# PantoMatrix/PantoMatrix

Hardware: NVIDIA H100
Metric: motion_frames_per_sec (higher is better)
Workload: dtype fp16x3 (two fp16 operand planes, 3 products, f32 accumulate)

## Files before the change

include/pm_emage.h:

```cpp
#ifndef PM_EMAGE_H
#define PM_EMAGE_H
#include <stdint.h>
#ifdef __cplusplus
extern "C" {
#endif

#define PM_ABI_VERSION 5
#define PM_FMT_F16 0x100
#define PM_TC_TILE_SHIFT 16
int pm_abi_version(void);
int pm_memset_async(void* ptr, int value, long long bytes, void* stream);
int pm_device_cc(void);

int pm_tapgemm_f32(const float* A, long long a_bs, int lda, int batch, int rows_in, int cin,
                   const float* W, const float* bias, int taps, int stride, int pad,
                   int rows_out, int cout,
                   const float* residual, long long r_bs, int ldr,
                   int act, float slope,
                   float* out, long long o_bs, int ldo, void* stream);

int pm_tapgemm_tc(const uint16_t* A, long long a_ps, long long a_bs, int lda, int batch, int rows_in, int cin,
                  const uint16_t* W, long long w_ps, int w_rows, int ldw, int taps, int pad, int nsplit,
                  const float* bias, int rows_out, int cout,
                  const float* residual, long long r_bs, int ldr,
                  int act, int act_cols, float slope, float acc_scale,
                  float* out_f32, long long o_bs, int ldo,
                  uint16_t* out_bf16, long long ob_ps, long long ob_bs, int ldob, int out_nsplit,
                  const void* prefetch, long long prefetch_bytes, void* stream);

int pm_split_bf16(const float* x, long long x_bs, int ldx, int batch, int rows, int ch,
                  uint16_t* out, long long o_ps, long long o_bs, int ldo, int nsplit, void* stream);

int pm_wav_stem_f32(const float* audio, long long a_bs, long long a_ws, int batch, int windows, int n_samples,
                    const float* w1, const float* b1, const float* wd, const float* bd, int cout,
                    int ksize, int stride, int pad, int rows_out, float slope,
                    float* y1, float* sc,
                    uint16_t* planes, long long p_ps, int p_ld, int p_nsplit, void* stream);

int pm_add_layernorm_f32(const float* x, const float* r, const float* gamma, const float* beta,
                         float* out, long long rows, int ch, float eps,
                         uint16_t* planes, long long p_ps, int p_ld, int p_nsplit, void* stream);

int pm_attention_f32(const float* Q, int ldq, const float* K, int ldk, const float* V, int ldv,
                     float* O, int ldo, int batch, int heads, int tq, int tk, int head_dim,
                     uint16_t* planes, long long p_ps, int p_ld, int p_nsplit, void* stream);

int pm_attention_tc(const uint16_t* Q, long long q_ps, long long q_bs, int ldq, int q_cols, int q_col0,
                    const uint16_t* K, long long k_ps, long long k_bs, int ldk, int k_cols, int k_col0,
                    const uint16_t* V, long long v_ps, long long v_bs, int ldv, int v_cols, int v_col0,
                    float* O, int ldo, int batch, int heads, int tq, int tk, int head_dim,
                    uint16_t* planes, long long p_ps, int p_ld, int p_nsplit, void* stream);

int pm_add_rows_f32(const float* x, const float* pe, const float* spk, int first, int second,
                    float* out, int batch, int rows, int ch,
                    uint16_t* planes, long long p_ps, int p_ld, int p_nsplit, void* stream);
int pm_add2_f32(const float* a, const float* b, float* out, long long n, int ch,
                uint16_t* planes, long long p_ps, int p_ld, int p_nsplit, void* stream);
int pm_add2_strided_f32(const float* a, long long lda, const float* b, long long ldb, float* out, long long ldo,
                        long long rows, long long ch,
                        uint16_t* planes, long long p_ps, int p_ld, int p_nsplit, void* stream);

int pm_window_input_f32(const float* motion, const float* mask, const float* seed, const float* mask_embedding,
                        float* out, int batch, int total_len, int start, int win_len, int pre, int ch, long long seed_bs,
                        uint16_t* planes, long long p_ps, int p_ld, int p_nsplit, void* stream);

int pm_l2_argmin_f32(const float* z, long long rows, int rows_per_batch, long long z_bs,
                     const float* codebook, const float* e2, int n_codes, int e_dim, long long* index, void* stream);
int pm_l2_argmin_tc(const float* z, long long rows, int rows_per_batch, long long z_bs,
                    const float* codebook, const float* e2, int n_codes, int e_dim, long long* index, int max_ctas,
                    void* stream);
int pm_l2_argmin_simt_f32(const float* z, long long rows, int rows_per_batch, long long z_bs,
                          const float* codebook, const float* e2, int n_codes, int e_dim, long long* index, void* stream);
int pm_row_argmax_f32(const float* x, long long rows, int ch, int ldx, int rows_per_batch, long long x_bs,
                      long long* index, int* nonfinite, void* stream);
int pm_gather_rows_f32(const float* codebook, long long n_table, const long long* index, long long rows, int ch,
                       float* out, uint16_t* planes, long long p_ps, int p_ld, int p_nsplit, void* stream);
int pm_row_sqnorm_f32(const float* x, int rows, int ch, float* out, void* stream);

int pm_pose_compose_f32(const float* face, const float* upper, const float* hands, const float* lower,
                        float* expression, float* axis_angle, float* motion4inf, long long bt, void* stream);

int pm_global_trans_f32(const float* rec, int ld, int vel_off, const float* ref_trans, int ref_bs, float dt,
                        float* trans, int batch, int t, void* stream);

int pm_resample_poly_f32(const void* pcm, int is_int16, long long in_bs, int batch, long long n_in, int channels,
                         const float* bank, int up, int down, int taps, long long n_pre_remove,
                         float* out, long long out_bs, void* stream);

int pm_lstm_bidir_f32(const float* xproj, long long x_bs, int ldx, const float* whh,
                      float* y, long long y_bs, int ldy, unsigned int* barrier,
                      int batch, int t, int hidden, void* stream);
int pm_lstm_cond_f32(const float* spk, long long n_spk, int spk_dim, const long long* speaker_id,
// ... 11 lines not shown
```

pantomatrix_b200/csrc/pm_tapgemm_tc.cu:

```cuda
#include <cuda.h>
#include <stdio.h>
#include <stdlib.h>

#include <cstring>
#include "pm_common.cuh"
#include "../../include/pm_emage.h"


namespace {

constexpr int BM = 128;
constexpr int BK = 64;
constexpr int MMA_K = 16;
constexpr int A_TILE_BYTES = BM * BK * 2;
constexpr int PRODUCER_THREADS = 128;
constexpr int CONSUMER_THREADS = 256;
constexpr int NUM_THREADS = PRODUCER_THREADS + CONSUMER_THREADS;
constexpr int PRODUCER_REGS = 40, CONSUMER_REGS = 232;
static_assert(PRODUCER_THREADS * PRODUCER_REGS + CONSUMER_THREADS * CONSUMER_REGS == (65536 / NUM_THREADS & ~7) * NUM_THREADS,
              "the setmaxnreg split must use exactly the launch's register pool");
constexpr int STAMP_WARP = PRODUCER_THREADS / 32;
constexpr int MAX_STAGES = 8;
constexpr int RING_KB = 200;

struct TcParams {
  int taps, pad, nsplit, kblocks;
  int rows_out, cout, batch;
  int R, NB;
  int w_rows;
  const float* bias;
  const float* residual; long long r_bs; int ldr;
  int act, act_cols; float slope;
  float* out_f32; long long o_bs; int ldo;
  __nv_bfloat16* out_bf16; long long ob_ps, ob_bs; int ldob; int out_nsplit;
  int stages;
  const uint8_t* prefetch; long long prefetch_bytes;
  float acc_scale;
};

#ifdef PM_TC_TIMING
__device__ unsigned long long pm_tc_stamps[4096 * 8];
#define PM_STAMP(i)                                                                                              \
  do {                                                                                                           \
    if ((threadIdx.x & 31) == 0) {                                                                               \
      const unsigned cta_ = (blockIdx.z * gridDim.y + blockIdx.y) * gridDim.x + blockIdx.x;                      \
      if (cta_ < 4096) pm_tc_stamps[cta_ * 8 + (i)] = (unsigned long long)clock64();                             \
    }                                                                                                            \
  } while (0)
#else
#define PM_STAMP(i) do {} while (0)
#endif

#include "pm_tc_ptx.cuh"

template <int BN, bool F16>
__device__ __forceinline__ void mma_k16(float (&d)[BN / 2], uint64_t a, uint64_t b) {
  static_assert(BN == 64 || BN == 128, "64- or 128-column tiles (see pm_tapgemm_tc)");
  if constexpr (BN == 64) wgmma_m64n64k16<!F16>(d, a, b);
  else wgmma_m64n128k16<!F16>(d, a, b);
}

template <int BN, bool F16, int NSPLIT>
__device__ __forceinline__ void mma_kblock(float (&main)[BN / 2], float (&corr)[BN / 2], uint64_t a0, uint64_t w0) {
  constexpr uint64_t A_PL = A_TILE_BYTES >> 4, W_PL = (BN * BK * 2) >> 4, K_ST = (MMA_K * 2) >> 4;
  if constexpr (NSPLIT == 3) {
#pragma unroll
    for (int k = 0; k < BK / MMA_K; ++k) mma_k16<BN, F16>(corr, a0 + k * K_ST, w0 + 2 * W_PL + k * K_ST);
#pragma unroll
    for (int k = 0; k < BK / MMA_K; ++k) mma_k16<BN, F16>(corr, a0 + A_PL + k * K_ST, w0 + W_PL + k * K_ST);
#pragma unroll
    for (int k = 0; k < BK / MMA_K; ++k) mma_k16<BN, F16>(corr, a0 + 2 * A_PL + k * K_ST, w0 + k * K_ST);
  }
  if constexpr (NSPLIT >= 2) {
#pragma unroll
    for (int k = 0; k < BK / MMA_K; ++k) mma_k16<BN, F16>(corr, a0 + k * K_ST, w0 + W_PL + k * K_ST);
#pragma unroll
    for (int k = 0; k < BK / MMA_K; ++k) mma_k16<BN, F16>(corr, a0 + A_PL + k * K_ST, w0 + k * K_ST);
  }
#pragma unroll
  for (int k = 0; k < BK / MMA_K; ++k) mma_k16<BN, F16>(main, a0 + k * K_ST, w0 + k * K_ST);
}

template <int BN, bool F16, int NSPLIT>
__global__ void __launch_bounds__(NUM_THREADS, 1) tapgemm_tc_kernel(const __grid_constant__ CUtensorMap map_a,
                                                                  const __grid_constant__ CUtensorMap map_w,
                                                                  const TcParams p) {
  constexpr int W_TILE_BYTES = BN * BK * 2;
  constexpr int NACC = BN / 2;
  constexpr int ST = BN + 8;

  extern __shared__ __align__(1024) uint8_t smem_raw[];
  uint8_t* tiles = reinterpret_cast<uint8_t*>((reinterpret_cast<uintptr_t>(smem_raw) + 1023) & ~uintptr_t(1023));
  const int stage_bytes = p.nsplit * (A_TILE_BYTES + W_TILE_BYTES);
  const int ring_bytes = p.stages * stage_bytes > BM * ST * 4 ? p.stages * stage_bytes : BM * ST * 4;
  uint64_t* bars = reinterpret_cast<uint64_t*>(tiles + ring_bytes);
  uint64_t* full_bar = bars;
  uint64_t* empty_bar = bars + MAX_STAGES;

  const int warp = threadIdx.x >> 5, lane = threadIdx.x & 31;
  if (warp == STAMP_WARP) PM_STAMP(0);
  const int l0 = blockIdx.x * p.R;
  const int n0 = blockIdx.y * BN;
  const int b0 = blockIdx.z * p.NB;
  const int n_iter = p.taps * p.kblocks;

  if (threadIdx.x == 0) {
    asm volatile("prefetch.tensormap [%0];" ::"l"(&map_a) : "memory");
    asm volatile("prefetch.tensormap [%0];" ::"l"(&map_w) : "memory");
    for (int s = 0; s < p.stages; ++s) {
      mbar_init(smem_u32(&full_bar[s]), 1);
      mbar_init(smem_u32(&empty_bar[s]), 2);
    }
    asm volatile("fence.mbarrier_init.release.cluster;" ::: "memory");
  }
  __syncthreads();
  if (warp == STAMP_WARP) PM_STAMP(1);

  if (warp < PRODUCER_THREADS / 32) {
    setmaxnreg_dec<PRODUCER_REGS>();
    if (warp == 1 && lane == 0 && p.prefetch) {
      const long long ncta = (long long)gridDim.x * gridDim.y * gridDim.z;
      const long long cta = ((long long)blockIdx.z * gridDim.y + blockIdx.y) * gridDim.x + blockIdx.x;
      long long share = ((p.prefetch_bytes + ncta - 1) / ncta + 127) & ~127LL;
      long long off = cta * share;
      long long end = off + share < p.prefetch_bytes ? off + share : p.prefetch_bytes;
      end &= ~15LL;
      for (; off < end; off += 16384) {
        const uint32_t n = (uint32_t)(end - off < 16384 ? end - off : 16384);
        asm volatile("cp.async.bulk.prefetch.L2.global [%0], %1;" ::"l"(p.prefetch + off), "r"(n) : "memory");
      }
    }
    if (warp != 0) return;
    const uint32_t tx = (uint32_t)stage_bytes;
    int s = 0, tap = 0, kb = 0;
    uint32_t ph = 0;
    for (int it = 0; it < n_iter; ++it) {
      mbar_wait_fast(smem_u32(&empty_bar[s]), ph ^ 1u);
      if (elect_one()) {
        const uint32_t bar = smem_u32(&full_bar[s]);
        uint8_t* st = tiles + (size_t)s * stage_bytes;
        mbar_expect_tx(bar, tx);
        for (int pl = 0; pl < p.nsplit; ++pl) {
          tma_load_4d(smem_u32(st + pl * A_TILE_BYTES), &map_a, bar, kb * BK, l0 + tap - p.pad, b0, pl);
          tma_load_3d(smem_u32(st + p.nsplit * A_TILE_BYTES + pl * W_TILE_BYTES), &map_w, bar, kb * BK, tap * p.w_rows + n0, pl);
        }
      }
      __syncwarp();
      if (++s == p.stages) { s = 0; ph ^= 1u; }
      if (++kb == p.kblocks) { kb = 0; ++tap; }
    }
    return;
  }

  setmaxnreg_inc<CONSUMER_REGS>();
  const int ct = threadIdx.x - PRODUCER_THREADS;
  const int wg = ct >> 7;
  float acc0[NACC], acc1[NACC], accc[NACC];
#pragma unroll
  for (int i = 0; i < NACC; ++i) { acc0[i] = 0.f; acc1[i] = 0.f; accc[i] = 0.f; }
  {
    const uint32_t tiles_u32 = smem_u32(tiles);
    int s = 0;
    uint32_t ph = 0;
    int prev = -1;
    auto kblock = [&](float (&main)[NACC]) {
      mbar_wait_fast(smem_u32(&full_bar[s]), ph);
      if (prev < 0 && warp == STAMP_WARP) PM_STAMP(2);
      const uint32_t a_base = tiles_u32 + (uint32_t)s * (uint32_t)stage_bytes + (uint32_t)wg * (64 * 128);
      const uint32_t w_base = tiles_u32 + (uint32_t)s * (uint32_t)stage_bytes + (uint32_t)(NSPLIT * A_TILE_BYTES);
      wgmma_fence();
      mma_kblock<BN, F16, NSPLIT>(main, accc, gmma_desc(GMMA_DESC_K_SW128, a_base), gmma_desc(GMMA_DESC_K_SW128, w_base));
      wgmma_commit();
      wgmma_wait<1>();
      if (prev >= 0 && ct % 128 == 0) mbar_arrive(smem_u32(&empty_bar[prev]));
      prev = s;
      if (++s == p.stages) { s = 0; ph ^= 1u; }
    };
    int it = 0;
    for (; it + 1 < n_iter; it += 2) {
      kblock(acc0);
      kblock(acc1);
    }
    if (it < n_iter) kblock(acc0);
    if (warp == STAMP_WARP) PM_STAMP(3);
    wgmma_wait<0>();
    if (warp == STAMP_WARP) PM_STAMP(4);
    wgmma_fence_regs(acc0);
    wgmma_fence_regs(acc1);
    wgmma_fence_regs(accc);
  }
  named_bar_sync(1, CONSUMER_THREADS);
  {
    const int wq = warp & 3, t4 = lane & 3;
    const int r0 = wg * 64 + wq * 16 + (lane >> 2);
    float* stg = reinterpret_cast<float*>(tiles);
#pragma unroll
    for (int i = 0; i < NACC / 4; ++i) {
      const int c = 8 * i + 2 * t4;
#pragma unroll
      for (int h = 0; h < 2; ++h) {
        float v0 = acc0[4 * i + 2 * h] + acc1[4 * i + 2 * h];
        float v1 = acc0[4 * i + 2 * h + 1] + acc1[4 * i + 2 * h + 1];
        v0 += accc[4 * i + 2 * h];
        v1 += accc[4 * i + 2 * h + 1];
        if constexpr (F16) { v0 *= p.acc_scale; v1 *= p.acc_scale; }
        *reinterpret_cast<float2*>(stg + (r0 + 8 * h) * ST + c) = make_float2(v0, v1);
      }
    }
  }
  named_bar_sync(1, CONSUMER_THREADS);

  const bool vec_f = p.out_f32 && ((p.ldo & 3) == 0) && ((reinterpret_cast<uintptr_t>(p.out_f32) & 15) == 0) && ((p.o_bs & 3) == 0);
  const bool vec_r = p.residual && ((p.ldr & 3) == 0) && ((reinterpret_cast<uintptr_t>(p.residual) & 15) == 0) && ((p.r_bs & 3) == 0);
  const bool vec_b = p.out_bf16 && ((p.ldob & 3) == 0) && ((reinterpret_cast<uintptr_t>(p.out_bf16) & 7) == 0) &&
                     ((p.ob_bs & 3) == 0) && ((p.ob_ps & 3) == 0);
  const bool all_vec = (!p.out_f32 || vec_f) && (!p.residual || vec_r) && (!p.out_bf16 || vec_b);
  const float act_slope = p.act == PM_ACT_NONE ? 1.f : (p.act == PM_ACT_RELU ? 0.f : p.slope);
  const int r_shift = 31 - __clz(p.R);
  constexpr int C4 = BN / 4;
  const float* stg = reinterpret_cast<const float*>(tiles);
#pragma unroll 1
  for (int item = ct; item < BM * C4; item += CONSUMER_THREADS) {
    const int rt = item / C4, c = (item % C4) * 4;
    const int b = b0 + (rt >> r_shift), l = l0 + (rt & (p.R - 1));
    const int n = n0 + c;
    if (b >= p.batch || l >= p.rows_out || n >= p.cout) continue;
    const float4 x4 = *reinterpret_cast<const float4*>(stg + rt * ST + c);
    const long long of = (long long)b * p.o_bs + (long long)l * p.ldo;
    const long long orr = (long long)b * p.r_bs + (long long)l * p.ldr;
    const PmPlanes P{p.out_bf16 ? p.out_bf16 + (long long)b * p.ob_bs + (long long)l * p.ldob : nullptr,
                     p.ob_ps, p.ldob, p.out_nsplit};
    if (all_vec && n + 4 <= p.cout) {
      float4 x = x4;
      if (p.bias) { x.x += __ldg(p.bias + n); x.y += __ldg(p.bias + n + 1); x.z += __ldg(p.bias + n + 2); x.w += __ldg(p.bias + n + 3); }
      if (p.residual) {
        const float4 t = *reinterpret_cast<const float4*>(p.residual + orr + n);
        x.x += t.x; x.y += t.y; x.z += t.z; x.w += t.w;
      }
      x.x = x.x < 0.f ? (n < p.act_cols ? act_slope : 1.f) * x.x : x.x;
      x.y = x.y < 0.f ? (n + 1 < p.act_cols ? act_slope : 1.f) * x.y : x.y;
      x.z = x.z < 0.f ? (n + 2 < p.act_cols ? act_slope : 1.f) * x.z : x.z;
      x.w = x.w < 0.f ? (n + 3 < p.act_cols ? act_slope : 1.f) * x.w : x.w;
      if (p.out_f32) *reinterpret_cast<float4*>(p.out_f32 + of + n) = x;
      if (P.ptr) pm_store_planes4_t<F16>(P, 0, n, x);
    } else {
      const float xs[4] = {x4.x, x4.y, x4.z, x4.w};
#pragma unroll
      for (int k = 0; k < 4; ++k) {
        if (n + k >= p.cout) break;
        float y = xs[k];
        if (p.bias) y += __ldg(p.bias + n + k);
        if (p.residual) y += p.residual[orr + n + k];
        y = y < 0.f ? (n + k < p.act_cols ? act_slope : 1.f) * y : y;
        if (p.out_f32) p.out_f32[of + n + k] = y;
        if (P.ptr) pm_store_planes_t<F16>(P, 0, n + k, y);
      }
    }
  }
  if (warp == STAMP_WARP) PM_STAMP(5);
#ifdef PM_TC_TIMING
  named_bar_sync(1, CONSUMER_THREADS);
#endif
  if (warp == STAMP_WARP) PM_STAMP(6);
}

template <bool VEC, bool F16>
__global__ void __launch_bounds__(256) split_bf16_kernel(const float* __restrict__ x, long long x_bs, int ldx, int rows,
                                                         int ch, __nv_bfloat16* __restrict__ out, long long o_ps,
                                                         long long o_bs, int ldo, int nsplit) {
  const int b = blockIdx.y;
  const float* __restrict__ xb = x + (long long)b * x_bs;
  __nv_bfloat16* __restrict__ ob = out + (long long)b * o_bs;
  if (VEC) {
    const int ch4 = ch >> 2;
    const long long total = (long long)rows * ch4;
    for (long long i = (long long)blockIdx.x * blockDim.x + threadIdx.x; i < total; i += (long long)gridDim.x * blockDim.x) {
      const int r = (int)(i / ch4), c4 = (int)(i - (long long)r * ch4);
      const float4 v = *reinterpret_cast<const float4*>(xb + (long long)r * ldx + 4 * c4);
      const PmPlanes P{ob, o_ps, ldo, nsplit};
      pm_store_planes4_t<F16>(P, r, 4 * c4, v);
    }
  } else {
    const long long total = (long long)rows * ch;
    for (long long i = (long long)blockIdx.x * blockDim.x + threadIdx.x; i < total; i += (long long)gridDim.x * blockDim.x) {
      const int r = (int)(i / ch), c = (int)(i - (long long)r * ch);
      const PmPlanes P{ob, o_ps, ldo, nsplit};
      pm_store_planes_t<F16>(P, r, c, xb[(long long)r * ldx + c]);
    }
  }
}

template <int BN, bool F16, int NSPLIT>
int launch(const CUtensorMap& ma, const CUtensorMap& mw, TcParams& p, dim3 grid, cudaStream_t st) {
  const int stage_bytes = p.nsplit * (A_TILE_BYTES + BN * BK * 2);
  int stages = RING_KB * 1024 / stage_bytes;
  if (stages > MAX_STAGES) stages = MAX_STAGES;
  if (stages < 2) return PM_EUNSUPPORTED;
  p.stages = stages;
  const int staging = BM * (BN + 8) * 4;
  const size_t ring = (size_t)stages * stage_bytes > (size_t)staging ? (size_t)stages * stage_bytes : (size_t)staging;
  const size_t smem = ring + 1024  + 2 * MAX_STAGES * sizeof(uint64_t);
  static unsigned long long configured = 0;
  if (pm_first_use_on_device(configured)) {
    cudaError_t e = cudaFuncSetAttribute(tapgemm_tc_kernel<BN, F16, NSPLIT>, cudaFuncAttributeMaxDynamicSharedMemorySize, 227 * 1024);
    if (e != cudaSuccess) { configured = 0; return (int)e; }
  }
  tapgemm_tc_kernel<BN, F16, NSPLIT><<<grid, NUM_THREADS, smem, st>>>(ma, mw, p);
  PM_LAUNCH_CHECK();
}

template <int BN>
int launch_fmt(const CUtensorMap& ma, const CUtensorMap& mw, TcParams& p, dim3 grid, cudaStream_t st, bool f16) {
  if (f16) {
    if (p.nsplit == 1) return launch<BN, true, 1>(ma, mw, p, grid, st);
    if (p.nsplit == 2) return launch<BN, true, 2>(ma, mw, p, grid, st);
    return launch<BN, true, 3>(ma, mw, p, grid, st);
  }
  if (p.nsplit == 1) return launch<BN, false, 1>(ma, mw, p, grid, st);
  if (p.nsplit == 2) return launch<BN, false, 2>(ma, mw, p, grid, st);
  return launch<BN, false, 3>(ma, mw, p, grid, st);
}

int pick_bn(long long row_tiles, int cout, int w_rows, int sms) {
  if (cout <= 64 || w_rows % 128) return 64;
  const long long waves64 = (row_tiles * pm_cdiv(cout, 64) + sms - 1) / sms;
  const long long waves128 = (row_tiles * pm_cdiv(cout, 128) + sms - 1) / sms;
  return waves128 * 14 <= waves64 * 10 ? 128 : 64;
}

}

extern "C" int pm_tapgemm_tc(const uint16_t* A, long long a_ps, long long a_bs, int lda, int batch, int rows_in, int cin,
                             const uint16_t* W, long long w_ps, int w_rows, int ldw, int taps, int pad, int nsplit,
                             const float* bias, int rows_out, int cout,
                             const float* residual, long long r_bs, int ldr,
                             int act, int act_cols, float slope, float acc_scale,
                             float* out_f32, long long o_bs, int ldo,
                             uint16_t* out_bf16, long long ob_ps, long long ob_bs, int ldob, int out_nsplit,
                             const void* prefetch, long long prefetch_bytes, void* stream) {
  PM_REQUIRE(A && W && (out_f32 || out_bf16));
  const int tile = (nsplit >> PM_TC_TILE_SHIFT) & 0xff;
  PM_TAKE_FMT(nsplit, f16);
  PM_TAKE_FMT(out_nsplit, out_f16);
  PM_REQUIRE(!out_bf16 || out_f16 == f16);
  PM_REQUIRE(f16 || acc_scale == 1.0f);
  PM_REQUIRE(!prefetch || (prefetch_bytes >= 0 && (reinterpret_cast<uintptr_t>(prefetch) & 15) == 0));
  PM_REQUIRE(batch > 0 && rows_in > 0 && rows_out > 0 && cin > 0 && cout > 0 && taps > 0);
  PM_REQUIRE(nsplit >= 1 && nsplit <= 3 && (!out_bf16 || (out_nsplit >= 1 && out_nsplit <= 3)));
  PM_REQUIRE(act >= PM_ACT_NONE && act <= PM_ACT_LEAKY);
  PM_REQUIRE((reinterpret_cast<uintptr_t>(A) & 15) == 0 && (reinterpret_cast<uintptr_t>(W) & 15) == 0);
  PM_REQUIRE((lda & 7) == 0 && (ldw & 7) == 0 && lda >= cin && ldw >= cin && w_rows >= cout);
  PM_REQUIRE(batch == 1 || (a_bs & 7) == 0);
  PM_REQUIRE(nsplit == 1 || ((a_ps & 7) == 0 && (w_ps & 7) == 0));
  PM_REQUIRE(!out_f32 || ldo >= cout);
  PM_REQUIRE(!out_bf16 || ldob >= cout);
  PM_REQUIRE(!residual || ldr >= cout);

  int R = 128;
  if (rows_out <= 64 && batch > 1) { R = 16; while (R < rows_out) R <<= 1; }
  const int NB = 128 / R;
  PM_REQUIRE(tile <= 2 && w_rows % 64 == 0 && (tile != 2 || w_rows % 128 == 0));
  int BNsel = tile == 1 ? 64 : 128;
  if (tile == 0) {
    int dev = 0, sms = 0;
    cudaError_t e = cudaGetDevice(&dev);
    if (e == cudaSuccess) e = cudaDeviceGetAttribute(&sms, cudaDevAttrMultiProcessorCount, dev);
    if (e != cudaSuccess) return (int)e;
    BNsel = pick_bn((long long)pm_cdiv(rows_out, R) * pm_cdiv(batch, NB), cout, w_rows, sms);
  }

  TcParams p;
  p.taps = taps; p.pad = pad; p.nsplit = nsplit; p.kblocks = (cin + BK - 1) / BK;
  p.rows_out = rows_out; p.cout = cout; p.batch = batch; p.R = R; p.NB = NB; p.w_rows = w_rows;
  p.bias = bias; p.residual = residual; p.r_bs = r_bs; p.ldr = ldr;
  p.act = act; p.act_cols = act_cols <= 0 ? cout : act_cols; p.slope = slope;
  p.out_f32 = out_f32; p.o_bs = o_bs; p.ldo = ldo;
  p.out_bf16 = reinterpret_cast<__nv_bfloat16*>(out_bf16); p.ob_ps = ob_ps; p.ob_bs = ob_bs; p.ldob = ldob;
  p.out_nsplit = out_bf16 ? out_nsplit : 0;
  p.stages = 0;
  p.prefetch = static_cast<const uint8_t*>(prefetch);
  p.prefetch_bytes = prefetch ? prefetch_bytes : 0;
  p.acc_scale = acc_scale;
  CUtensorMap ma, mw;
  {
    const long long bs_el = batch > 1 ? a_bs : (long long)rows_in * lda;
    const long long ps_el = nsplit > 1 ? a_ps : bs_el * batch;
    cuuint64_t dims[4] = {(cuuint64_t)cin, (cuuint64_t)rows_in, (cuuint64_t)batch, (cuuint64_t)nsplit};
    cuuint64_t strides[3] = {(cuuint64_t)lda * 2, (cuuint64_t)bs_el * 2, (cuuint64_t)ps_el * 2};
    cuuint32_t box[4] = {(cuuint32_t)BK, (cuuint32_t)R, (cuuint32_t)NB, 1};
    if (!encode_map(&ma, A, 4, dims, strides, box, f16)) return PM_EBADARG;
  }
  {
    const long long ps_el = nsplit > 1 ? w_ps : (long long)taps * w_rows * ldw;
    cuuint64_t dims[3] = {(cuuint64_t)cin, (cuuint64_t)taps * w_rows, (cuuint64_t)nsplit};
    cuuint64_t strides[2] = {(cuuint64_t)ldw * 2, (cuuint64_t)ps_el * 2};
    cuuint32_t box[3] = {(cuuint32_t)BK, (cuuint32_t)BNsel, 1};
    if (!encode_map(&mw, W, 3, dims, strides, box, f16)) return PM_EBADARG;
  }
  dim3 grid(pm_cdiv(rows_out, R), pm_cdiv(cout, BNsel), pm_cdiv(batch, NB));
  PM_REQUIRE(grid.z <= 65535 && grid.y <= 65535);
  const cudaStream_t st = (cudaStream_t)stream;
  if (BNsel == 128) return launch_fmt<128>(ma, mw, p, grid, st, f16);
  return launch_fmt<64>(ma, mw, p, grid, st, f16);
}

#ifdef PM_TC_TIMING
extern "C" int pm_tc_timing_reset() {
  cudaError_t e = cudaDeviceSynchronize();
  if (e != cudaSuccess) return (int)e;
  void* d = nullptr;
  e = cudaGetSymbolAddress(&d, pm_tc_stamps);
  if (e != cudaSuccess) return (int)e;
  return (int)cudaMemset(d, 0, sizeof(unsigned long long) * 4096 * 8);
}
extern "C" int pm_tc_timing_read(unsigned long long* host) {
  cudaError_t e = cudaDeviceSynchronize();
  if (e != cudaSuccess) return (int)e;
  return (int)cudaMemcpyFromSymbol(host, pm_tc_stamps, sizeof(unsigned long long) * 4096 * 8);
}
#endif

extern "C" int pm_split_bf16(const float* x, long long x_bs, int ldx, int batch, int rows, int ch,
                             uint16_t* out, long long o_ps, long long o_bs, int ldo, int nsplit, void* stream) {
  PM_TAKE_FMT(nsplit, f16);
  PM_REQUIRE(x && out && batch >= 0 && rows >= 0 && ch > 0 && ldx >= ch && ldo >= ch && nsplit >= 1 && nsplit <= 3);
  if ((long long)batch * rows == 0) return PM_OK;
  PM_REQUIRE(batch <= 65535);
  const bool vec = (ch & 3) == 0 && (ldx & 3) == 0 && (x_bs & 3) == 0 && (ldo & 3) == 0 && (o_bs & 3) == 0 &&
                   (o_ps & 3) == 0 && (reinterpret_cast<uintptr_t>(x) & 15) == 0 && (reinterpret_cast<uintptr_t>(out) & 7) == 0;
  const long long work = (long long)rows * (vec ? ch / 4 : ch);
  long long gx = (work + 255) / 256;
  const long long cap = batch >= 132 * 4 ? 1 : (132 * 8 + batch - 1) / batch;
  if (gx > cap) gx = cap;
  dim3 grid((unsigned)gx, batch);
  __nv_bfloat16* o = reinterpret_cast<__nv_bfloat16*>(out);
  cudaStream_t st = (cudaStream_t)stream;
  if (f16) {
    if (vec) split_bf16_kernel<true, true><<<grid, 256, 0, st>>>(x, x_bs, ldx, rows, ch, o, o_ps, o_bs, ldo, nsplit);
    else split_bf16_kernel<false, true><<<grid, 256, 0, st>>>(x, x_bs, ldx, rows, ch, o, o_ps, o_bs, ldo, nsplit);
  } else {
    if (vec) split_bf16_kernel<true, false><<<grid, 256, 0, st>>>(x, x_bs, ldx, rows, ch, o, o_ps, o_bs, ldo, nsplit);
    else split_bf16_kernel<false, false><<<grid, 256, 0, st>>>(x, x_bs, ldx, rows, ch, o, o_ps, o_bs, ldo, nsplit);
  }
  PM_LAUNCH_CHECK();
}
```

pantomatrix_b200/ops.py:

```python
from __future__ import annotations

import math

import torch

from . import _lib

ACT_NONE, ACT_RELU, ACT_LEAKY = 0, 1, 2
ROW_NONE, ROW_PE, ROW_SPK = 0, 1, 2

launch_count = 0

FMT_F16 = 0x100
TC_TILE_SHIFT = 16
F16_ACT_SCALE = 64.0
_PLANE_DTYPE = torch.bfloat16


def set_plane_format(name: str) -> None:
    global _PLANE_DTYPE
    _PLANE_DTYPE = {"bf16": torch.bfloat16, "fp16": torch.float16}[name]


def plane_format() -> str:
    return "fp16" if _PLANE_DTYPE == torch.float16 else "bf16"


def _fmt_bit(t) -> int:
    return FMT_F16 if t.dtype == torch.float16 else 0


def _stream() -> int:
    return torch.cuda.current_stream().cuda_stream


def _ptr(t) -> int | None:
    return None if t is None else t.data_ptr()


def _chk(t: torch.Tensor, dtype=torch.float32):
    if not t.is_cuda:
        raise _lib.PmError("pantomatrix_b200 ops need CUDA tensors (no CPU fallback)")
    if t.dtype != dtype:
        raise _lib.PmError(f"expected {dtype}, got {t.dtype}")
    if t.dim() and t.stride(-1) != 1 and t.shape[-1] != 1:
        raise _lib.PmError("innermost dimension must be contiguous")
    return t


def _call(name, *args):
    global launch_count
    launch_count += 1
    _lib.call(name, *args)


def _bs_ld(t: torch.Tensor):
    return (t.stride(0) if t.shape[0] > 1 else t.shape[1] * t.stride(1)), t.stride(1)


def tapgemm(a, w, bias, *, rows_out=None, stride=1, pad=0, act=ACT_NONE, slope=0.0, residual=None, out=None):
    _chk(a), _chk(w)
    batch, rows_in, cin = a.shape
    taps, cout, cin_w = w.shape
    assert cin_w == cin and w.is_contiguous(), (w.shape, a.shape)
    if rows_out is None:
        rows_out = (rows_in + 2 * pad - taps) // stride + 1
    if out is None:
        out = torch.empty(batch, rows_out, cout, device=a.device, dtype=torch.float32)
    else:
        assert out.shape == (batch, rows_out, cout), (out.shape, (batch, rows_out, cout))
    _chk(out)
    if residual is not None:
        _chk(residual)
        assert residual.shape == out.shape
    if (taps == 1 and pad == 0 and stride == 1 and batch > 1 and a.stride(0) == rows_in * a.stride(1)
            and out.stride(0) == rows_out * out.stride(1)
            and (residual is None or residual.stride(0) == rows_out * residual.stride(1))):
        a = a.reshape(1, batch * rows_in, cin) if a.is_contiguous() else a.as_strided(
            (1, batch * rows_in, cin), (0, a.stride(1), 1), a.storage_offset())
        flat = lambda t: t.as_strided((1, batch * rows_out, cout), (0, t.stride(1), 1), t.storage_offset())
        out_v = flat(out)
        res_v = flat(residual) if residual is not None else None
        batch_k, rows_in_k, rows_out_k = 1, batch * rows_in, batch * rows_out
    else:
        out_v, res_v, batch_k, rows_in_k, rows_out_k = out, residual, batch, rows_in, rows_out
    a_bs, lda = _bs_ld(a)
    o_bs, ldo = _bs_ld(out_v)
    r_bs, ldr = _bs_ld(res_v) if res_v is not None else (0, 0)
    _call("pm_tapgemm_f32", a.data_ptr(), a_bs, lda, batch_k, rows_in_k, cin,
          w.data_ptr(), _ptr(bias), taps, stride, pad, rows_out_k, cout,
          _ptr(res_v), r_bs, ldr, act, float(slope), out_v.data_ptr(), o_bs, ldo, _stream())
    return out


def wav_stem(audio, a_bs, a_ws, batch, windows, n_samples, w1, b1, wd, bd, *, stride, pad, slope, offset=0, nsplit=0):
    _chk(audio)
    cout, ks = w1.shape
# ... 261 lines not shown
    expression = torch.empty(bs, t, 100, device=device, dtype=torch.float32)
    axis_angle = torch.empty(bs, t, 165, device=device, dtype=torch.float32)
    motion4inf = torch.empty(bs, t, 337, device=device, dtype=torch.float32)
    _call("pm_pose_compose_f32", _ptr(face), _ptr(upper), _ptr(hands), _ptr(lower), expression.data_ptr(),
          axis_angle.data_ptr(), motion4inf.data_ptr(), bs * t, _stream())
    return expression, axis_angle, motion4inf


def global_trans(rec, ref_trans, dt, vel_off=54):
    _chk(rec), _chk(ref_trans)
    assert rec.is_contiguous()
    bs, t, ld = rec.shape
    assert ref_trans.shape == (bs, 3)
    trans = torch.empty(bs, t, 3, device=rec.device, dtype=torch.float32)
    _call("pm_global_trans_f32", rec.data_ptr(), ld, vel_off, ref_trans.data_ptr(), ref_trans.stride(0), float(dt),
          trans.data_ptr(), bs, t, _stream())
    return trans




def _round_up(x, m):
    return (x + m - 1) // m * m


class Planes:
    __slots__ = ("t", "rows", "ch", "slack")

    def __init__(self, t, rows, ch, slack=0):
        self.t, self.rows, self.ch, self.slack = t, rows, ch, slack

    def flat(self):
        ns, b, r, ld = self.t.shape
        assert self.t.stride(1) == r * self.t.stride(2)
        return Planes(self.t.as_strided((ns, 1, b * r, ld), (self.t.stride(0), b * r * self.t.stride(2), self.t.stride(2), 1),
                                        self.t.storage_offset()), b * r, self.ch, self.slack)

    @property
    def nsplit(self):
        return self.t.shape[0]

    @property
    def batch(self):
        return self.t.shape[1]


def split_bf16(x, nsplit, slack_rows=0):
    _chk(x)
    batch, rows, ch = x.shape
    pl = _new_planes(nsplit, (batch, rows), ch, x.device, slack_rows)
    x_bs, ldx = _bs_ld(x)
    _call("pm_split_bf16", x.data_ptr(), x_bs, ldx, batch, rows, ch, pl.t.data_ptr(), pl.t.stride(0), pl.t.stride(1),
          pl.t.stride(2), nsplit | _fmt_bit(pl.t), _stream())
    return pl


class PackedW:
    __slots__ = ("t", "taps", "cout", "cin", "w_rows", "ldw", "acc_scale")

    def __init__(self, w, nsplit):
        taps, cout, cin = w.shape
        bn = 64 if cout <= 64 else 128
        self.taps, self.cout, self.cin = taps, cout, cin
        self.w_rows, self.ldw = _round_up(cout, bn), _round_up(cin, 8)
        full = torch.zeros(taps, self.w_rows, self.ldw, device=w.device, dtype=torch.float32)
        full[:, :cout, :cin] = w
        self.acc_scale = 1.0
        if _PLANE_DTYPE == torch.float16:
            m = float(full.abs().max())
            if m > 0.0 and math.isfinite(m):
                k = math.floor(math.log2(32768.0 / m))
                full = full * (2.0 ** k)
                self.acc_scale = 2.0 ** -k
            self.acc_scale /= F16_ACT_SCALE
        planes, rem = [], full
        for _ in range(nsplit):
            p = rem.to(_PLANE_DTYPE)
            planes.append(p)
            rem = rem - p.float()
        self.t = torch.stack(planes).contiguous()


def tapgemm_tc(a: Planes, w: PackedW, bias, *, rows_in=None, rows_out, pad=0, act=ACT_NONE, act_cols=0, slope=0.0,
               residual=None, want_f32=True, out_nsplit=0, out=None, a_view=None, out_slack=0, prefetch=None, tile=0):
    t = a.t
    nsplit, batch = t.shape[0], t.shape[1]
    assert nsplit == w.t.shape[0] and t.dtype == w.t.dtype, "A and W must use the same split and plane format"
    fmt = _fmt_bit(t)
    rows_a, cin, lda = (a.rows, a.ch, t.stride(2)) if a_view is None else a_view
    if rows_in is not None:
        rows_a = rows_in
    assert cin == w.cin, (cin, w.cin)
    assert tile in (0, 64, 128), tile
    cout = w.cout
    dev = t.device
    out_f = None
    if want_f32:
        out_f = out if out is not None else torch.empty(batch, rows_out, cout, device=dev, dtype=torch.float32)
        assert out_f.shape == (batch, rows_out, cout)
    o_bs, ldo = _bs_ld(out_f) if out_f is not None else (0, 0)
    out_p = None
    if out_nsplit:
        out_p = _new_planes(out_nsplit, (batch, rows_out), cout, dev, out_slack, dtype=t.dtype)
    r_bs, ldr = _bs_ld(residual) if residual is not None else (0, 0)
    if residual is not None:
        _chk(residual)
        assert residual.shape == (batch, rows_out, cout)
    _call("pm_tapgemm_tc", t.data_ptr(), t.stride(0), t.stride(1), lda, batch, rows_a, cin,
          w.t.data_ptr(), w.t.stride(0), w.w_rows, w.ldw, w.taps, pad, nsplit | fmt | (tile // 64) << TC_TILE_SHIFT,
          _ptr(bias), rows_out, cout, _ptr(residual), r_bs, ldr, act, act_cols, float(slope), float(w.acc_scale),
          _ptr(out_f), o_bs, ldo,
          None if out_p is None else out_p.t.data_ptr(), 0 if out_p is None else out_p.t.stride(0),
          0 if out_p is None else out_p.t.stride(1), 0 if out_p is None else out_p.t.stride(2),
          out_nsplit | (fmt if out_nsplit else 0),
          None if prefetch is None else prefetch.data_ptr(),
          0 if prefetch is None else prefetch.numel() * prefetch.element_size(), _stream())
    return out_f, out_p




def lstm_bidir(xproj, whh, barrier, hidden):
    _chk(xproj), _chk(whh)
    assert xproj.is_contiguous() and whh.is_contiguous() and whh.shape == (2, 4 * hidden, hidden)
    batch, t, w = xproj.shape
    assert w == 8 * hidden
    y = torch.empty(batch, t, 2 * hidden, device=xproj.device, dtype=torch.float32)
    _call("pm_lstm_bidir_f32", xproj.data_ptr(), xproj.stride(0), xproj.stride(1), whh.data_ptr(), y.data_ptr(),
          y.stride(0), y.stride(1), barrier.data_ptr(), batch, t, hidden, _stream())
    return y


def rot6d_to_aa(rot6d, slot, n_sel):
    _chk(rot6d)
    assert rot6d.is_contiguous() and rot6d.shape[-1] == n_sel * 6
    rows = rot6d.numel() // (n_sel * 6)
    out = torch.empty(*rot6d.shape[:-1], 165, device=rot6d.device, dtype=torch.float32)
    _call("pm_rot6d_to_aa_f32", rot6d.data_ptr(), rows, n_sel, slot.data_ptr(), out.data_ptr(), _stream())
    return out


def softmax2_mix(sel, c1, c2, out=None):
    _chk(sel), _chk(c1), _chk(c2)
    assert sel.is_contiguous() and c1.is_contiguous() and c2.is_contiguous() and sel.shape[-1] == 2
    ch = c1.shape[-1]
    rows = c1.numel() // ch
    if out is None:
        out = torch.empty_like(c1)
    _call("pm_softmax2_mix_f32", sel.data_ptr(), c1.data_ptr(), c2.data_ptr(), out.data_ptr(), rows, ch, out.stride(-2), _stream())
    return out
```

Baseline: 247,300.

## Stage conv input halo once in shared memory and reuse across taps

```diff
diff --git a/include/pm_emage.h b/include/pm_emage.h
--- a/include/pm_emage.h
+++ b/include/pm_emage.h
@@ -8,6 +8,7 @@
 #define PM_ABI_VERSION 5
 #define PM_FMT_F16 0x100
 #define PM_TC_TILE_SHIFT 16
+#define PM_TC_STAGING_SHIFT 20
 int pm_abi_version(void);
 int pm_memset_async(void* ptr, int value, long long bytes, void* stream);
 int pm_device_cc(void);
diff --git a/pantomatrix_b200/csrc/pm_tapgemm_tc.cu b/pantomatrix_b200/csrc/pm_tapgemm_tc.cu
--- a/pantomatrix_b200/csrc/pm_tapgemm_tc.cu
+++ b/pantomatrix_b200/csrc/pm_tapgemm_tc.cu
@@ -9,10 +9,9 @@
 
 namespace {
 
-constexpr int BM = 128;
 constexpr int BK = 64;
 constexpr int MMA_K = 16;
-constexpr int A_TILE_BYTES = BM * BK * 2;
+constexpr int A_TILE_BYTES = 128 * BK * 2;
 constexpr int PRODUCER_THREADS = 128;
 constexpr int CONSUMER_THREADS = 256;
 constexpr int NUM_THREADS = PRODUCER_THREADS + CONSUMER_THREADS;
@@ -22,11 +21,14 @@
 constexpr int STAMP_WARP = PRODUCER_THREADS / 32;
 constexpr int MAX_STAGES = 8;
 constexpr int RING_KB = 200;
+constexpr int SMEM_MAX = 227 * 1024;
+constexpr int SMEM_SLACK = 1024 + (2 * MAX_STAGES + 1) * 8;
 
 struct TcParams {
   int taps, pad, nsplit, kblocks;
   int rows_out, cout, batch;
   int R, NB;
+  int halo_rows, halo_box;
   int w_rows;
   const float* bias;
   const float* residual; long long r_bs; int ldr;
@@ -53,49 +55,63 @@
 
 #include "pm_tc_ptx.cuh"
 
-template <int BN, bool F16>
-__device__ __forceinline__ void mma_k16(float (&d)[BN / 2], uint64_t a, uint64_t b) {
+template <int BN, bool F16, bool TRANS, int NA>
+__device__ __forceinline__ void mma_k16(float (&d)[NA], uint64_t a, uint64_t w) {
   static_assert(BN == 64 || BN == 128, "64- or 128-column tiles (see pm_tapgemm_tc)");
-  if constexpr (BN == 64) wgmma_m64n64k16<!F16>(d, a, b);
-  else wgmma_m64n128k16<!F16>(d, a, b);
-}
-
-template <int BN, bool F16, int NSPLIT>
-__device__ __forceinline__ void mma_kblock(float (&main)[BN / 2], float (&corr)[BN / 2], uint64_t a0, uint64_t w0) {
-  constexpr uint64_t A_PL = A_TILE_BYTES >> 4, W_PL = (BN * BK * 2) >> 4, K_ST = (MMA_K * 2) >> 4;
+  if constexpr (TRANS) wgmma_m64n128k16<!F16>(d, w, a);
+  else if constexpr (BN == 64) wgmma_m64n64k16<!F16>(d, a, w);
+  else wgmma_m64n128k16<!F16>(d, a, w);
+}
+
+template <int BN, bool F16, int NSPLIT, bool TRANS, int NA>
+__device__ __forceinline__ void mma_kblock(float (&main)[NA], float (&corr)[NA], uint64_t a0, uint64_t w0, uint64_t A_PL) {
+  constexpr uint64_t W_PL = (BN * BK * 2) >> 4, K_ST = (MMA_K * 2) >> 4;
   if constexpr (NSPLIT == 3) {
 #pragma unroll
-    for (int k = 0; k < BK / MMA_K; ++k) mma_k16<BN, F16>(corr, a0 + k * K_ST, w0 + 2 * W_PL + k * K_ST);
-#pragma unroll
-    for (int k = 0; k < BK / MMA_K; ++k) mma_k16<BN, F16>(corr, a0 + A_PL + k * K_ST, w0 + W_PL + k * K_ST);
-#pragma unroll
-    for (int k = 0; k < BK / MMA_K; ++k) mma_k16<BN, F16>(corr, a0 + 2 * A_PL + k * K_ST, w0 + k * K_ST);
+    for (int k = 0; k < BK / MMA_K; ++k) mma_k16<BN, F16, TRANS>(corr, a0 + k * K_ST, w0 + 2 * W_PL + k * K_ST);
+#pragma unroll
+    for (int k = 0; k < BK / MMA_K; ++k) mma_k16<BN, F16, TRANS>(corr, a0 + A_PL + k * K_ST, w0 + W_PL + k * K_ST);
+#pragma unroll
+    for (int k = 0; k < BK / MMA_K; ++k) mma_k16<BN, F16, TRANS>(corr, a0 + 2 * A_PL + k * K_ST, w0 + k * K_ST);
   }
   if constexpr (NSPLIT >= 2) {
 #pragma unroll
-    for (int k = 0; k < BK / MMA_K; ++k) mma_k16<BN, F16>(corr, a0 + k * K_ST, w0 + W_PL + k * K_ST);
-#pragma unroll
-    for (int k = 0; k < BK / MMA_K; ++k) mma_k16<BN, F16>(corr, a0 + A_PL + k * K_ST, w0 + k * K_ST);
-  }
-#pragma unroll
-  for (int k = 0; k < BK / MMA_K; ++k) mma_k16<BN, F16>(main, a0 + k * K_ST, w0 + k * K_ST);
-}
-
-template <int BN, bool F16, int NSPLIT>
+    for (int k = 0; k < BK / MMA_K; ++k) mma_k16<BN, F16, TRANS>(corr, a0 + k * K_ST, w0 + W_PL + k * K_ST);
+#pragma unroll
+    for (int k = 0; k < BK / MMA_K; ++k) mma_k16<BN, F16, TRANS>(corr, a0 + A_PL + k * K_ST, w0 + k * K_ST);
+  }
+#pragma unroll
+  for (int k = 0; k < BK / MMA_K; ++k) mma_k16<BN, F16, TRANS>(main, a0 + k * K_ST, w0 + k * K_ST);
+}
+
+__host__ __device__ constexpr int stage_bytes_of(int nsplit, int bn, bool halo) {
+  return nsplit * ((halo ? 0 : A_TILE_BYTES) + bn * BK * 2);
+}
+__host__ __device__ constexpr int staging_bytes_of(int bm, int bn) { return bm * (bn + 8) * 4; }
+
+template <int BN, bool F16, int NSPLIT, int BM>
 __global__ void __launch_bounds__(NUM_THREADS, 1) tapgemm_tc_kernel(const __grid_constant__ CUtensorMap map_a,
                                                                   const __grid_constant__ CUtensorMap map_w,
                                                                   const TcParams p) {
+  static_assert(BM == 128 || (BM == 256 && BN == 64), "256-row tiles: 64 columns (the same accumulator registers)");
+  constexpr bool TRANS = BM == 256;
   constexpr int W_TILE_BYTES = BN * BK * 2;
-  constexpr int NACC = BN / 2;
+  constexpr int NACC = TRANS ? 64 : BN / 2;
   constexpr int ST = BN + 8;
 
   extern __shared__ __align__(1024) uint8_t smem_raw[];
   uint8_t* tiles = reinterpret_cast<uint8_t*>((reinterpret_cast<uintptr_t>(smem_raw) + 1023) & ~uintptr_t(1023));
-  const int stage_bytes = p.nsplit * (A_TILE_BYTES + W_TILE_BYTES);
-  const int ring_bytes = p.stages * stage_bytes > BM * ST * 4 ? p.stages * stage_bytes : BM * ST * 4;
-  uint64_t* bars = reinterpret_cast<uint64_t*>(tiles + ring_bytes);
+  const bool halo = p.halo_rows > 0;
+  const int res_plane = p.halo_rows * 128;
+  const int res_bytes = halo ? p.kblocks * NSPLIT * res_plane : 0;
+  const int a_bytes = halo ? 0 : NSPLIT * A_TILE_BYTES;
+  const int stage_bytes = stage_bytes_of(NSPLIT, BN, halo);
+  const int used = res_bytes + p.stages * stage_bytes;
+  uint64_t* bars = reinterpret_cast<uint64_t*>(tiles + (used > staging_bytes_of(BM, BN) ? used : staging_bytes_of(BM, BN)));
   uint64_t* full_bar = bars;
   uint64_t* empty_bar = bars + MAX_STAGES;
+  uint64_t* res_bar = bars + 2 * MAX_STAGES;
+  uint8_t* ring = tiles + res_bytes;
 
   const int warp = threadIdx.x >> 5, lane = threadIdx.x & 31;
   if (warp == STAMP_WARP) PM_STAMP(0);
@@ -111,6 +127,7 @@
       mbar_init(smem_u32(&full_bar[s]), 1);
       mbar_init(smem_u32(&empty_bar[s]), 2);
     }
+    mbar_init(smem_u32(res_bar), 1);
     asm volatile("fence.mbarrier_init.release.cluster;" ::: "memory");
   }
   __syncthreads();
@@ -131,6 +148,18 @@
       }
     }
     if (warp != 0) return;
+    if (halo) {
+      if (elect_one()) {
+        const uint32_t bar = smem_u32(res_bar);
+        mbar_expect_tx(bar, (uint32_t)res_bytes);
+        for (int kb = 0; kb < p.kblocks; ++kb)
+          for (int pl = 0; pl < NSPLIT; ++pl)
+            for (int r = 0; r < p.halo_rows; r += p.halo_box)
+              tma_load_4d(smem_u32(tiles + (kb * NSPLIT + pl) * res_plane + r * 128), &map_a, bar, kb * BK,
+                          l0 - p.pad + r, b0, pl);
+      }
+      __syncwarp();
+    }
     const uint32_t tx = (uint32_t)stage_bytes;
     int s = 0, tap = 0, kb = 0;
     uint32_t ph = 0;
@@ -138,11 +167,11 @@
       mbar_wait_fast(smem_u32(&empty_bar[s]), ph ^ 1u);
       if (elect_one()) {
         const uint32_t bar = smem_u32(&full_bar[s]);
-        uint8_t* st = tiles + (size_t)s * stage_bytes;
+        uint8_t* st = ring + (size_t)s * stage_bytes;
         mbar_expect_tx(bar, tx);
-        for (int pl = 0; pl < p.nsplit; ++pl) {
-          tma_load_4d(smem_u32(st + pl * A_TILE_BYTES), &map_a, bar, kb * BK, l0 + tap - p.pad, b0, pl);
-          tma_load_3d(smem_u32(st + p.nsplit * A_TILE_BYTES + pl * W_TILE_BYTES), &map_w, bar, kb * BK, tap * p.w_rows + n0, pl);
+        for (int pl = 0; pl < NSPLIT; ++pl) {
+          if (!halo) tma_load_4d(smem_u32(st + pl * A_TILE_BYTES), &map_a, bar, kb * BK, l0 + tap - p.pad, b0, pl);
+          tma_load_3d(smem_u32(st + a_bytes + pl * W_TILE_BYTES), &map_w, bar, kb * BK, tap * p.w_rows + n0, pl);
         }
       }
       __syncwarp();
@@ -159,22 +188,27 @@
 #pragma unroll
   for (int i = 0; i < NACC; ++i) { acc0[i] = 0.f; acc1[i] = 0.f; accc[i] = 0.f; }
   {
-    const uint32_t tiles_u32 = smem_u32(tiles);
-    int s = 0;
+    const uint32_t tiles_u32 = smem_u32(tiles), ring_u32 = smem_u32(ring);
+    const uint64_t a_pl = (uint64_t)((halo ? res_plane : A_TILE_BYTES) >> 4);
+    int s = 0, tap = 0, kb = 0;
     uint32_t ph = 0;
     int prev = -1;
+    if (halo) mbar_wait(smem_u32(res_bar), 0);
     auto kblock = [&](float (&main)[NACC]) {
       mbar_wait_fast(smem_u32(&full_bar[s]), ph);
       if (prev < 0 && warp == STAMP_WARP) PM_STAMP(2);
-      const uint32_t a_base = tiles_u32 + (uint32_t)s * (uint32_t)stage_bytes + (uint32_t)wg * (64 * 128);
-      const uint32_t w_base = tiles_u32 + (uint32_t)s * (uint32_t)stage_bytes + (uint32_t)(NSPLIT * A_TILE_BYTES);
+      const uint32_t a_base = halo ? tiles_u32 + (uint32_t)(kb * NSPLIT * res_plane) + (uint32_t)(wg * (BM / 2) + tap) * 128
+                                   : ring_u32 + (uint32_t)s * (uint32_t)stage_bytes + (uint32_t)wg * (64 * 128);
+      const uint32_t w_base = ring_u32 + (uint32_t)s * (uint32_t)stage_bytes + (uint32_t)a_bytes;
       wgmma_fence();
-      mma_kblock<BN, F16, NSPLIT>(main, accc, gmma_desc(GMMA_DESC_K_SW128, a_base), gmma_desc(GMMA_DESC_K_SW128, w_base));
+      mma_kblock<BN, F16, NSPLIT, TRANS>(main, accc, gmma_desc(GMMA_DESC_K_SW128, a_base),
+                                         gmma_desc(GMMA_DESC_K_SW128, w_base), a_pl);
       wgmma_commit();
       wgmma_wait<1>();
       if (prev >= 0 && ct % 128 == 0) mbar_arrive(smem_u32(&empty_bar[prev]));
       prev = s;
       if (++s == p.stages) { s = 0; ph ^= 1u; }
+      if (++kb == p.kblocks) { kb = 0; ++tap; }
     };
     int it = 0;
     for (; it + 1 < n_iter; it += 2) {
@@ -192,8 +226,8 @@
   named_bar_sync(1, CONSUMER_THREADS);
   {
     const int wq = warp & 3, t4 = lane & 3;
-    const int r0 = wg * 64 + wq * 16 + (lane >> 2);
     float* stg = reinterpret_cast<float*>(tiles);
+    const int q = wq * 16 + (lane >> 2);
 #pragma unroll
     for (int i = 0; i < NACC / 4; ++i) {
       const int c = 8 * i + 2 * t4;
@@ -204,7 +238,13 @@
         v0 += accc[4 * i + 2 * h];
         v1 += accc[4 * i + 2 * h + 1];
         if constexpr (F16) { v0 *= p.acc_scale; v1 *= p.acc_scale; }
-        *reinterpret_cast<float2*>(stg + (r0 + 8 * h) * ST + c) = make_float2(v0, v1);
+        if constexpr (TRANS) {
+          const int r = wg * 128 + c;
+          stg[r * ST + q + 8 * h] = v0;
+          stg[(r + 1) * ST + q + 8 * h] = v1;
+        } else {
+          *reinterpret_cast<float2*>(stg + (wg * 64 + q + 8 * h) * ST + c) = make_float2(v0, v1);
+        }
       }
     }
   }
@@ -290,35 +330,40 @@
   }
 }
 
-template <int BN, bool F16, int NSPLIT>
+int ring_stages(int nsplit, int bn, int kblocks, int halo_rows) {
+  const bool halo = halo_rows > 0;
+  const int sb = stage_bytes_of(nsplit, bn, halo);
+  int stages = halo ? (SMEM_MAX - SMEM_SLACK - kblocks * nsplit * halo_rows * 128) / sb : RING_KB * 1024 / sb;
+  if (stages > MAX_STAGES) stages = MAX_STAGES;
+  return stages >= (halo ? 3 : 2) ? stages : 0;
+}
+
+template <int BN, bool F16, int NSPLIT, int BM>
 int launch(const CUtensorMap& ma, const CUtensorMap& mw, TcParams& p, dim3 grid, cudaStream_t st) {
-  const int stage_bytes = p.nsplit * (A_TILE_BYTES + BN * BK * 2);
-  int stages = RING_KB * 1024 / stage_bytes;
-  if (stages > MAX_STAGES) stages = MAX_STAGES;
-  if (stages < 2) return PM_EUNSUPPORTED;
-  p.stages = stages;
-  const int staging = BM * (BN + 8) * 4;
-  const size_t ring = (size_t)stages * stage_bytes > (size_t)staging ? (size_t)stages * stage_bytes : (size_t)staging;
-  const size_t smem = ring + 1024  + 2 * MAX_STAGES * sizeof(uint64_t);
+  p.stages = ring_stages(NSPLIT, BN, p.kblocks, p.halo_rows);
+  if (p.stages == 0) return PM_EUNSUPPORTED;
+  const size_t used = (size_t)p.kblocks * NSPLIT * p.halo_rows * 128 + (size_t)p.stages * stage_bytes_of(NSPLIT, BN, p.halo_rows > 0);
+  const size_t staging = staging_bytes_of(BM, BN);
+  const size_t smem = (used > staging ? used : staging) + SMEM_SLACK;
   static unsigned long long configured = 0;
   if (pm_first_use_on_device(configured)) {
-    cudaError_t e = cudaFuncSetAttribute(tapgemm_tc_kernel<BN, F16, NSPLIT>, cudaFuncAttributeMaxDynamicSharedMemorySize, 227 * 1024);
+    cudaError_t e = cudaFuncSetAttribute(tapgemm_tc_kernel<BN, F16, NSPLIT, BM>, cudaFuncAttributeMaxDynamicSharedMemorySize, SMEM_MAX);
     if (e != cudaSuccess) { configured = 0; return (int)e; }
   }
-  tapgemm_tc_kernel<BN, F16, NSPLIT><<<grid, NUM_THREADS, smem, st>>>(ma, mw, p);
+  tapgemm_tc_kernel<BN, F16, NSPLIT, BM><<<grid, NUM_THREADS, smem, st>>>(ma, mw, p);
   PM_LAUNCH_CHECK();
 }
 
-template <int BN>
+template <int BN, int BM>
 int launch_fmt(const CUtensorMap& ma, const CUtensorMap& mw, TcParams& p, dim3 grid, cudaStream_t st, bool f16) {
   if (f16) {
-    if (p.nsplit == 1) return launch<BN, true, 1>(ma, mw, p, grid, st);
-    if (p.nsplit == 2) return launch<BN, true, 2>(ma, mw, p, grid, st);
-    return launch<BN, true, 3>(ma, mw, p, grid, st);
-  }
-  if (p.nsplit == 1) return launch<BN, false, 1>(ma, mw, p, grid, st);
-  if (p.nsplit == 2) return launch<BN, false, 2>(ma, mw, p, grid, st);
-  return launch<BN, false, 3>(ma, mw, p, grid, st);
+    if (p.nsplit == 1) return launch<BN, true, 1, BM>(ma, mw, p, grid, st);
+    if (p.nsplit == 2) return launch<BN, true, 2, BM>(ma, mw, p, grid, st);
+    return launch<BN, true, 3, BM>(ma, mw, p, grid, st);
+  }
+  if (p.nsplit == 1) return launch<BN, false, 1, BM>(ma, mw, p, grid, st);
+  if (p.nsplit == 2) return launch<BN, false, 2, BM>(ma, mw, p, grid, st);
+  return launch<BN, false, 3, BM>(ma, mw, p, grid, st);
 }
 
 int pick_bn(long long row_tiles, int cout, int w_rows, int sms) {
@@ -326,6 +371,17 @@
   const long long waves64 = (row_tiles * pm_cdiv(cout, 64) + sms - 1) / sms;
   const long long waves128 = (row_tiles * pm_cdiv(cout, 128) + sms - 1) / sms;
   return waves128 * 14 <= waves64 * 10 ? 128 : 64;
+}
+
+int halo_rows_of(int bm, int taps, int* box) {
+  const int need = bm + taps - 1, nbox = need > 256 ? 2 : 1;
+  *box = (pm_cdiv(need, nbox) + 7) & ~7;
+  return *box <= 256 ? nbox * *box : 0;
+}
+bool halo_fits(int R, int bm, int bn, int taps, int kblocks, int nsplit) {
+  int box = 0;
+  const int rows = halo_rows_of(bm, taps, &box);
+  return R == 128 && rows > 0 && ring_stages(nsplit, bn, kblocks, rows) > 0;
 }
 
 }
@@ -339,7 +395,8 @@
                              uint16_t* out_bf16, long long ob_ps, long long ob_bs, int ldob, int out_nsplit,
                              const void* prefetch, long long prefetch_bytes, void* stream) {
   PM_REQUIRE(A && W && (out_f32 || out_bf16));
-  const int tile = (nsplit >> PM_TC_TILE_SHIFT) & 0xff;
+  const int tile = (nsplit >> PM_TC_TILE_SHIFT) & 0xf;
+  const int staging = (nsplit >> PM_TC_STAGING_SHIFT) & 0xf;
   PM_TAKE_FMT(nsplit, f16);
   PM_TAKE_FMT(out_nsplit, out_f16);
   PM_REQUIRE(!out_bf16 || out_f16 == f16);
@@ -358,20 +415,40 @@
 
   int R = 128;
   if (rows_out <= 64 && batch > 1) { R = 16; while (R < rows_out) R <<= 1; }
-  const int NB = 128 / R;
-  PM_REQUIRE(tile <= 2 && w_rows % 64 == 0 && (tile != 2 || w_rows % 128 == 0));
+  PM_REQUIRE(tile <= 2 && staging <= 3 && w_rows % 64 == 0 && (tile != 2 || w_rows % 128 == 0));
+  int dev = 0, sms = 0;
+  cudaError_t e = cudaGetDevice(&dev);
+  if (e == cudaSuccess) e = cudaDeviceGetAttribute(&sms, cudaDevAttrMultiProcessorCount, dev);
+  if (e != cudaSuccess) return (int)e;
+  const int kblocks = (cin + BK - 1) / BK;
   int BNsel = tile == 1 ? 64 : 128;
-  if (tile == 0) {
-    int dev = 0, sms = 0;
-    cudaError_t e = cudaGetDevice(&dev);
-    if (e == cudaSuccess) e = cudaDeviceGetAttribute(&sms, cudaDevAttrMultiProcessorCount, dev);
-    if (e != cudaSuccess) return (int)e;
-    BNsel = pick_bn((long long)pm_cdiv(rows_out, R) * pm_cdiv(batch, NB), cout, w_rows, sms);
-  }
+  if (tile == 0) BNsel = pick_bn((long long)pm_cdiv(rows_out, R) * pm_cdiv(batch, 128 / R), cout, w_rows, sms);
+  bool halo = false;
+  int BM = 128;
+  if (staging == 0) {
+    halo = taps >= 3 && (long long)pm_cdiv(rows_out, 128) * batch * pm_cdiv(cout, BNsel) >= sms &&
+           halo_fits(R, 128, BNsel, taps, kblocks, nsplit);
+    if (halo && BNsel == 64 && halo_fits(R, 256, 64, taps, kblocks, nsplit) &&
+        (long long)pm_cdiv(rows_out, 256) * batch >= 3LL * sms)
+      BM = 256;
+  } else if (staging >= 2) {
+    halo = true;
+    BM = staging == 3 ? 256 : 128;
+    if (BM == 256) {
+      PM_REQUIRE(tile != 2);
+      BNsel = 64;
+    }
+    PM_REQUIRE(halo_fits(R, BM, BNsel, taps, kblocks, nsplit));
+  }
+  if (BM == 256) R = 256;
+  const int NB = BM / R;
+  int halo_box = 0;
+  const int halo_rows = halo ? halo_rows_of(BM, taps, &halo_box) : 0;
 
   TcParams p;
-  p.taps = taps; p.pad = pad; p.nsplit = nsplit; p.kblocks = (cin + BK - 1) / BK;
+  p.taps = taps; p.pad = pad; p.nsplit = nsplit; p.kblocks = kblocks;
   p.rows_out = rows_out; p.cout = cout; p.batch = batch; p.R = R; p.NB = NB; p.w_rows = w_rows;
+  p.halo_rows = halo_rows; p.halo_box = halo_box;
   p.bias = bias; p.residual = residual; p.r_bs = r_bs; p.ldr = ldr;
   p.act = act; p.act_cols = act_cols <= 0 ? cout : act_cols; p.slope = slope;
   p.out_f32 = out_f32; p.o_bs = o_bs; p.ldo = ldo;
@@ -387,7 +464,7 @@
     const long long ps_el = nsplit > 1 ? a_ps : bs_el * batch;
     cuuint64_t dims[4] = {(cuuint64_t)cin, (cuuint64_t)rows_in, (cuuint64_t)batch, (cuuint64_t)nsplit};
     cuuint64_t strides[3] = {(cuuint64_t)lda * 2, (cuuint64_t)bs_el * 2, (cuuint64_t)ps_el * 2};
-    cuuint32_t box[4] = {(cuuint32_t)BK, (cuuint32_t)R, (cuuint32_t)NB, 1};
+    cuuint32_t box[4] = {(cuuint32_t)BK, (cuuint32_t)(halo ? halo_box : R), (cuuint32_t)(halo ? 1 : NB), 1};
     if (!encode_map(&ma, A, 4, dims, strides, box, f16)) return PM_EBADARG;
   }
   {
@@ -400,8 +477,9 @@
   dim3 grid(pm_cdiv(rows_out, R), pm_cdiv(cout, BNsel), pm_cdiv(batch, NB));
   PM_REQUIRE(grid.z <= 65535 && grid.y <= 65535);
   const cudaStream_t st = (cudaStream_t)stream;
-  if (BNsel == 128) return launch_fmt<128>(ma, mw, p, grid, st, f16);
-  return launch_fmt<64>(ma, mw, p, grid, st, f16);
+  if (BM == 256) return launch_fmt<64, 256>(ma, mw, p, grid, st, f16);
+  if (BNsel == 128) return launch_fmt<128, 128>(ma, mw, p, grid, st, f16);
+  return launch_fmt<64, 128>(ma, mw, p, grid, st, f16);
 }
 
 #ifdef PM_TC_TIMING
diff --git a/pantomatrix_b200/ops.py b/pantomatrix_b200/ops.py
--- a/pantomatrix_b200/ops.py
+++ b/pantomatrix_b200/ops.py
@@ -13,6 +13,8 @@
 
 FMT_F16 = 0x100
 TC_TILE_SHIFT = 16
+TC_STAGING_SHIFT = 20
+TC_STAGING = {None: 0, "tap": 1, "halo128": 2, "halo256": 3}
 F16_ACT_SCALE = 64.0
 _PLANE_DTYPE = torch.bfloat16
 
@@ -440,7 +442,8 @@
 
 
 def tapgemm_tc(a: Planes, w: PackedW, bias, *, rows_in=None, rows_out, pad=0, act=ACT_NONE, act_cols=0, slope=0.0,
-               residual=None, want_f32=True, out_nsplit=0, out=None, a_view=None, out_slack=0, prefetch=None, tile=0):
+               residual=None, want_f32=True, out_nsplit=0, out=None, a_view=None, out_slack=0, prefetch=None, tile=0,
+               staging=None):
     t = a.t
     nsplit, batch = t.shape[0], t.shape[1]
     assert nsplit == w.t.shape[0] and t.dtype == w.t.dtype, "A and W must use the same split and plane format"
@@ -450,6 +453,10 @@
         rows_a = rows_in
     assert cin == w.cin, (cin, w.cin)
     assert tile in (0, 64, 128), tile
+    if a_view is not None:
+        if staging not in (None, "tap"):
+            raise ValueError("halo staging is for stride-1 convs: strided views stage per tap")
+        staging = "tap"
     cout = w.cout
     dev = t.device
     out_f = None
@@ -465,7 +472,7 @@
         _chk(residual)
         assert residual.shape == (batch, rows_out, cout)
     _call("pm_tapgemm_tc", t.data_ptr(), t.stride(0), t.stride(1), lda, batch, rows_a, cin,
-          w.t.data_ptr(), w.t.stride(0), w.w_rows, w.ldw, w.taps, pad, nsplit | fmt | (tile // 64) << TC_TILE_SHIFT,
+          w.t.data_ptr(), w.t.stride(0), w.w_rows, w.ldw, w.taps, pad, nsplit | fmt | (tile // 64) << TC_TILE_SHIFT | TC_STAGING[staging] << TC_STAGING_SHIFT,
           _ptr(bias), rows_out, cout, _ptr(residual), r_bs, ldr, act, act_cols, float(slope), float(w.acc_scale),
           _ptr(out_f), o_bs, ldo,
           None if out_p is None else out_p.t.data_ptr(), 0 if out_p is None else out_p.t.stride(0),
```

Result: faster. 252,700, median of 6 (+2.2%).
